# Meowuu7/equi-articulated-pose

Measured on AMD Instinct MI355X. Metric: point-clouds/sec (4096 pts, 60 anchors) fwd+bwd, higher is better.
Workload: dtype f32; 1 GPU; 8 x 4096-pt synthetic laptop clouds per GPU, 3-block inter backbone 1->64->128->512 (NN=64,K=24,A=60), forward+backward+Adam; clouds_per_gpu=8, points=4096, anchors=60

## Files before the change

equi-articulated-pose_amd/csrc/so3_dense.hip:

```cpp
#include <atomic>
#include "common.h"
#include "device_prims.h"
#include <type_traits>

namespace {

typedef unsigned long long u64;
typedef const __attribute__((address_space(4))) unsigned long long *cu64p;

constexpr int KC_BK = 32;
constexpr int KC_LIST_BYTES = 4096;

__host__ __device__ __forceinline__ void dense_kr(int d, int ks, int &k, int &r) {
    const int g = d / (16 * ks), rem = d - g * 16 * ks;
    k = rem >> 4;
    r = 16 * g + (rem & 15);
}


__device__ __forceinline__ void split2(float x0, float x1, unsigned &h, unsigned &l) {
    asm("v_cvt_pk_f16_f32 %0, %2, %3\n\t"
        "v_fma_mixlo_f16 %1, %0, -1.0, %2 op_sel:[0,0,0] op_sel_hi:[1,0,0]\n\t"
        "v_fma_mixhi_f16 %1, %0, -1.0, %3 op_sel:[1,0,0] op_sel_hi:[1,0,0]"
        : "=&v"(h), "=&v"(l) : "v"(x0), "v"(x1));
}

__global__ __launch_bounds__(256) void dense_slots_kernel(int n_sup, int rp, int rows_ld, const int32_t *__restrict__ rows,
                                                          const int32_t *__restrict__ n_rows, int32_t *__restrict__ slot_of) {
    const int b = blockIdx.y, j = blockIdx.x * 256 + threadIdx.x;
    if (j >= min(n_rows[b], rp)) return;
    const int r = rows[(size_t)b * rows_ld + j];
    if ((unsigned)r < (unsigned)n_sup) slot_of[(size_t)b * n_sup + r] = j;
}

constexpr int MEMB_WORDS = 16;
constexpr int MEMB_WORDS_WIDE = 32;
constexpr int DENSE_MAX_ROWS = 32 * MEMB_WORDS_WIDE;
template <int W>
__global__ __launch_bounds__(256) void dense_member_kernel(int p, int n_sup, int nn, int rp, const int32_t *__restrict__ idx,
                                                           const int32_t *__restrict__ slot_of, unsigned *__restrict__ memb,
                                                           int32_t *__restrict__ flags) {
    __shared__ unsigned sw[256][W + 1];
    const int b = blockIdx.y, pt = blockIdx.x * 256 + threadIdx.x;
    if (pt >= p) return;
    unsigned *w = sw[threadIdx.x];
    for (int k = 0; k < W; ++k) w[k] = 0u;
    const int32_t *list = idx + ((size_t)b * p + pt) * nn;
    int valid = 0, bad = 0;
    for (int n = 0; n < nn; ++n) {
        const int i = list[n];
        if ((unsigned)i >= (unsigned)n_sup) continue;
        const int s = slot_of[(size_t)b * n_sup + i];
        if (s < 0 || s >= rp) { bad |= 2; continue; }
        ++valid;
        w[s >> 5] |= 1u << (s & 31);
    }
    int bits = 0;
    for (int k = 0; k < W; ++k) { bits += __popc(w[k]); memb[((size_t)b * p + pt) * W + k] = w[k]; }
    if (bits != valid) bad |= 1;
    if (bad) atomicOr(&flags[b], bad);
}

template <int W>
__global__ __launch_bounds__(256) void dense_mask_kernel(int p, int ks, int rp, int dir, int wtiles, int steps,
                                                         const unsigned *__restrict__ memb, unsigned *__restrict__ bits) {
    const int b = blockIdx.y, lane = threadIdx.x & 63, li = lane & 31, kg = lane >> 5;
    const long long wv = (long long)blockIdx.x * 4 + (threadIdx.x >> 6);
    if (wv >= (long long)wtiles * steps) return;
    const int wt = (int)(wv / steps), step = (int)(wv - (long long)wt * steps);
    const int nkr = ks * rp;
    unsigned word = 0;
    if (dir == 0 && (ks & 3) == 0) {
        const int g = (64 * wt) / (16 * ks), pt_own = 32 * step + li;
        const unsigned own = (pt_own < p && 2 * (g >> 1) < 2 * W) ? memb[((size_t)b * p + pt_own) * W + (g >> 1)] : 0u;
        const int sh = 16 * (g & 1) + (li & 15);
        const bool col0 = 64 * wt + li < nkr, col1 = 64 * wt + 32 + li < nkr;
#pragma unroll
        for (int tt = 0; tt < 2; ++tt)
#pragma unroll
            for (int e = 0; e < 8; ++e) {
                const unsigned wd = (unsigned)__shfl((int)own, 16 * tt + 8 * kg + e);
                const unsigned bit = (wd >> sh) & 1u;
                word |= (col0 ? bit : 0u) << (16 * tt + e);
                word |= (col1 ? bit : 0u) << (16 * tt + 8 + e);
            }
    } else if (dir == 1) {
        const int d0 = 32 * step, g = d0 / (16 * ks);
#pragma unroll
        for (int j = 0; j < 2; ++j) {
            const int pt = 64 * wt + 32 * j + li;
            const unsigned wd = (pt < p && (g >> 1) < W) ? memb[((size_t)b * p + pt) * W + (g >> 1)] : 0u;
            const unsigned byte = (wd >> (16 * (g & 1) + 8 * kg)) & 0xffu;
#pragma unroll
            for (int tt = 0; tt < 2; ++tt)
                if (d0 + 16 * tt < nkr) word |= byte << (16 * tt + 8 * j);
        }
    } else {
#pragma unroll
        for (int i = 0; i < 32; ++i) {
            const int tt = i >> 4, j = (i >> 3) & 1, e = i & 7;
            const int n = 64 * wt + 32 * j + (lane & 31);
            const int kk = 32 * step + 16 * tt + 8 * (lane >> 5) + e;
            const int pt = dir ? n : kk, kr = dir ? kk : n;
            if (pt < p && kr < nkr) {
                int k_, r;
                dense_kr(kr, ks, k_, r);
                word |= ((memb[((size_t)b * p + pt) * W + (r >> 5)] >> (r & 31)) & 1u) << i;
            }
        }
    }
    bits[(((size_t)b * wtiles + wt) * steps + step) * 64 + lane] = word;
}

template <int W>
__global__ __launch_bounds__(256) void dense_keys_kernel(long long total, const unsigned *__restrict__ memb,
                                                         std::conditional_t<W == MEMB_WORDS, int32_t, int64_t> *__restrict__ keys) {
    using UK = std::conditional_t<W == MEMB_WORDS, unsigned, u64>;
    const long long i = (long long)blockIdx.x * 256 + threadIdx.x;
    if (i >= total) return;
    const u32x4 *w = reinterpret_cast<const u32x4 *>(memb + i * W);
    UK key = 0;
#pragma unroll
    for (int q = 0; q < W / 4; ++q) {
        const u32x4 v = w[q];
#pragma unroll
        for (int e = 0; e < 4; ++e) {
            const int g = 2 * (4 * q + e);
            key |= (UK)((v[e] & 0xffffu) ? 1u : 0u) << g;
            key |= (UK)((v[e] >> 16) ? 1u : 0u) << (g + 1);
        }
    }
    keys[i] = (std::conditional_t<W == MEMB_WORDS, int32_t, int64_t>)key;
}

__global__ __launch_bounds__(256) void dense_steps_kernel(int KS, int blocks_n, int wtiles, int dir, int ks, int row_slots, int skip,
                                                          const int32_t *__restrict__ n_rows, const unsigned *__restrict__ bits,
                                                          int32_t *__restrict__ steps) {
    extern __shared__ int nz[];
    const int b = blockIdx.y, bn = blockIdx.x, t = threadIdx.x, lane = t & 63, wave = t >> 6;
    for (int i = t; i < KS; i += 256) nz[i] = 0;
    __syncthreads();
    int limit = KS;
    if (dir == 1 && n_rows != nullptr) limit = max(min(KS, ((min(n_rows[b], row_slots) + 15) & ~15) * ks / KC_BK), 1);
    if (skip) {
        const int wt = min(4 * bn + wave, wtiles - 1);
        const unsigned *src = bits + ((size_t)b * wtiles + wt) * (size_t)KS * 64 + lane;
        for (int s = 0; s < limit; s += 4) {
            unsigned v[4];
#pragma unroll
            for (int u = 0; u < 4; ++u) v[u] = (s + u < limit) ? src[(size_t)(s + u) * 64] : 0u;
#pragma unroll
            for (int u = 0; u < 4; ++u)
                if (__builtin_amdgcn_ballot_w64(v[u] != 0u) != 0ull && lane == 0 && s + u < limit) nz[s + u] = 1;
        }
    } else {
        for (int i = t; i < limit; i += 256) nz[i] = 1;
    }
    __syncthreads();
    if (t == 0) {
        int32_t *dst = steps + ((size_t)b * blocks_n + bn) * (size_t)(KS + 1);
        int n = 0;
        for (int i = 0; i < KS; ++i)
            if (nz[i]) dst[1 + n++] = i;
        if (n == 0) dst[1 + n++] = 0;
        dst[0] = n;
    }
}

__global__ __launch_bounds__(256) void dense_centre_kernel(int n, const float *__restrict__ xyz, float *__restrict__ centre) {
    __shared__ double s[3][256];
    const int b = blockIdx.x;
// ... 318 lines not shown
                        v[4 + e] = hi ? own : got;
                    }
                    const int r0 = rc0 + 32 * rt + 16 * half + 8 * kg;
                    if (r0 < rc0 + nrows) {
                        unsigned h[4], l[4];
#pragma unroll
                        for (int e = 0; e < 4; ++e) split2(v[2 * e], v[2 * e + 1], h[e], l[e]);
                        const int kb = (r0 >> 4) * ks + k;
                        u32x4 *dst = planes + (((size_t)z * kb_total + kb) * MT + mt) * 128 + li + 32 * kg;
                        dst[0] = (u32x4){h[0], h[1], h[2], h[3]};
                        dst[64] = (u32x4){l[0], l[1], l[2], l[3]};
                    }
                }
            }
        }
    }
}

__global__ __launch_bounds__(256) void dense_untranspose_kernel(int nb, int o_total, int p, int na, int p_dst, const int32_t *__restrict__ map,
                                                                const int32_t *__restrict__ pivot_pos,
                                                                const float *__restrict__ yt, float *__restrict__ y,
                                                                float *__restrict__ psum, float *__restrict__ psq) {
    extern __shared__ float tile[];
    __shared__ float red[2][256];
    const int chunks = (p + 63) >> 6, t = threadIdx.x;
    const int p0 = (int)(blockIdx.x % (unsigned)chunks) * 64, grp_ = (int)(blockIdx.x / (unsigned)chunks), o = grp_ % o_total, b = grp_ / o_total;
    const int nchunk_x = chunks, nb_z = nb;
    const int np = min(64, p - p0);
    const float pivot = psum ? yt[(size_t)o * p + (pivot_pos ? *pivot_pos : 0)] : 0.f;
    float s = 0.f, q = 0.f;
    for (int i = t; i < na * 64; i += 256) {
        const int a = i >> 6, pp = i & 63;
        if (pp < np) {
            const float v = yt[(((size_t)b * na + a) * o_total + o) * p + p0 + pp];
            tile[a * 65 + pp] = v;
            if (psum != nullptr && (map == nullptr || map[(size_t)b * p + p0 + pp] >= 0)) {
                const float d = v - pivot;
                s += d; q = fmaf(d, d, q);
            }
        }
    }
    red[0][t] = s; red[1][t] = q;
    __syncthreads();
    const int nq = na >> 2;
    float *rows_y = y + ((size_t)b * o_total + o) * (size_t)(map ? p_dst : p) * na;
    for (int i = t; i < np * nq; i += 256) {
        const int pp = i / nq, a4 = i - pp * nq;
        const int q = map ? map[(size_t)b * p + p0 + pp] : p0 + pp;
        if (map != nullptr && (unsigned)q >= (unsigned)p_dst) continue;
        const float *src = tile + (4 * a4) * 65 + pp;
        const f32x4 v = {src[0], src[65], src[130], src[195]};
        *reinterpret_cast<f32x4 *>(rows_y + (size_t)q * na + 4 * a4) = v;
    }
    if (psum == nullptr) return;
    for (int h = 128; h > 0; h >>= 1) {
        if (t < h) { red[0][t] += red[0][t + h]; red[1][t] += red[1][t + h]; }
        __syncthreads();
    }
    if (t == 0) {
        const size_t at = ((size_t)o * nb_z + b) * nchunk_x + (p0 >> 6);
        psum[at] = red[0][0]; psq[at] = red[1][0];
    }
}

constexpr int UT_PTS = 128;
__global__ __launch_bounds__(256, 5) void dense_untranspose_tile_kernel(int o_total, int p, int na, int p_dst, const int32_t *__restrict__ map,
                                                                     const float *__restrict__ yt, float *__restrict__ y,
                                                                     const float *__restrict__ bn_scale, const float *__restrict__ bn_shift, float slope) {
    constexpr int UT_LD = UT_PTS / 16;
    extern __shared__ float tile[];
    __shared__ int dst_row[UT_PTS];
    const int chunks = (p + UT_PTS - 1) / UT_PTS, t = threadIdx.x;
    unsigned bid = blockIdx.x;
    if (const unsigned n8 = gridDim.x / 8u; bid < 8u * n8) bid = (bid % 8u) * n8 + bid / 8u;
    const int p0 = (int)(bid % (unsigned)chunks) * UT_PTS, grp_ = (int)(bid / (unsigned)chunks), o = grp_ % o_total, b = grp_ / o_total;
    const int np = min(UT_PTS, p - p0);
    if (t < UT_PTS) dst_row[t] = t >= np ? -1 : map ? map[(size_t)b * p + p0 + t] : p0 + t;
    const size_t a_pitch = (size_t)o_total * p;
    const float *src = yt + ((size_t)b * na * o_total + o) * p + p0;
    if ((p & 3) == 0) {
        f32x4 v[UT_LD];
#pragma unroll
        for (int k = 0; k < UT_LD; ++k) {
            const int i = t + 256 * k, a = i / (UT_PTS / 4), c = 4 * (i % (UT_PTS / 4));
            if (a < na && c < np) v[k] = *reinterpret_cast<const f32x4 *>(src + (size_t)a * a_pitch + c);
        }
#pragma unroll
        for (int k = 0; k < UT_LD; ++k) {
            const int i = t + 256 * k, a = i / (UT_PTS / 4), c = 4 * (i % (UT_PTS / 4));
            if (a < na && c < np) *reinterpret_cast<f32x4 *>(tile + a * UT_PTS + ((c + 4 * ((a >> 2) & 7)) & (UT_PTS - 1))) = v[k];
        }
    } else {
        for (int i = t; i < na * UT_PTS; i += 256) {
            const int a = i / UT_PTS, c = i % UT_PTS;
            if (c < np) tile[a * UT_PTS + ((c + 4 * ((a >> 2) & 7)) & (UT_PTS - 1))] = src[(size_t)a * a_pitch + c];
        }
    }
    __syncthreads();
    const int nq = na >> 2, RG = 256 / nq, a4 = t % nq, rr = t / nq;
    if (rr >= RG) return;
    const int rows_dst = map ? p_dst : p, rot = 4 * (a4 & 7);
    const float *quad = tile + (4 * a4) * UT_PTS;
    float *rows_y = y + ((size_t)b * o_total + o) * (size_t)rows_dst * na + 4 * a4;
    float sc = 1.f, sh = 0.f;
    if (bn_scale != nullptr) { sc = bn_scale[o]; sh = bn_shift[o]; }
    for (int pp0 = rr; pp0 < np; pp0 += 4 * RG) {
        f32x4 v[4];
        int q[4];
#pragma unroll
        for (int u = 0; u < 4; ++u) {
            const int pp = min(pp0 + u * RG, UT_PTS - 1), c = (pp + rot) & (UT_PTS - 1);
            q[u] = pp0 + u * RG < np ? dst_row[pp] : -1;
            v[u] = (f32x4){quad[c], quad[UT_PTS + c], quad[2 * UT_PTS + c], quad[3 * UT_PTS + c]};
        }
#pragma unroll
        for (int u = 0; u < 4; ++u) {
            if ((unsigned)q[u] >= (unsigned)rows_dst) continue;
            if (bn_scale != nullptr) {
#pragma unroll
                for (int e = 0; e < 4; ++e) { const float w = fmaf(v[u][e], sc, sh); v[u][e] = w > 0.f ? w : w * slope; }
            }
            *reinterpret_cast<f32x4 *>(rows_y + (size_t)q[u] * na) = v[u];
        }
    }
}

__global__ __launch_bounds__(256) void dense_zero_tail_kernel(int rows_ok, int na, int rp, long long ldz, const int32_t *__restrict__ n_rows,
                                                              float *__restrict__ z) {
    const int b = blockIdx.y, row = blockIdx.x;
    const int r0 = (min(n_rows[b], rp) + 15) & ~15, tail = rp - r0;
    if (tail <= 0) return;
    float *dst = z + ((long long)b * rows_ok + row) * ldz;
    for (int e = threadIdx.x; e < na * tail; e += 256) {
        const int a = e / tail;
        dst[(long long)a * rp + r0 + (e - a * tail)] = 0.f;
    }
}

struct KcArgs {
    int MT, N, KS, na, zcount;
    int tiles_m, blocks_n, mask_tiles;
    const u32x4 *A;
    const float *scale;
    const f32x4 *strT; long long strB, strA;
    const f32x4 *colT; long long colB, colA;
    const unsigned *mask;
    float neg_inv_sigma;
    const int32_t *n_rows; int ks, trim;
    float *C; long long cB, cA, ldm; int rp; long long kstride;
    int row_slots;
    const int32_t *steps;
};

template <int MI>
__global__ __launch_bounds__(256, MI == 4 ? 2 : 1) void kc_gemm_kernel(KcArgs g) {
    static_assert(MI == 8 || MI == 4, "the DMA piece schedule below: 8 or 4 KB of the stored operand per wave and k-step");
    constexpr unsigned WB = MI * 1024u;
    constexpr unsigned SUB_A = MI * 2048u;
    constexpr unsigned STR_OFF = 2 * SUB_A;
    constexpr unsigned BIT_OFF = STR_OFF + 1024u;
    constexpr unsigned STAGE = BIT_OFF + 1024u;
    extern __shared__ __attribute__((aligned(16))) unsigned char smem[];

    const int per_z = g.tiles_m * g.blocks_n;
    int id = blockIdx.x, z, local;
    {
        const int groups = g.zcount / 8 * 8;
        if (id < groups * per_z) {
            const int xcd = id & 7, slot = id >> 3;
            z = (slot / per_z) * 8 + xcd;
            local = slot % per_z;
        } else {
            const int r = id - groups * per_z;
            z = groups + r / per_z;
            local = r % per_z;
        }
    }
    const int bm = local % g.tiles_m, bn = local / g.tiles_m;
    const int b = z / g.na, a = z - b * g.na;
    const int used = (g.trim == 1 || g.trim == 2) ? ((min(g.n_rows[b], g.row_slots) + 15) & ~15) * g.ks : 0;
    const int N = g.trim == 1 ? min(g.N, used) : g.N;
    if (256 * bn >= N) return;
    const int32_t *lstG = g.steps ? g.steps + ((size_t)b * g.blocks_n + bn) * (size_t)(g.KS + 1) : nullptr;
    const int KS = lstG ? __builtin_amdgcn_readfirstlane(lstG[0]) : (g.trim == 2 ? max(min(g.KS, used / KC_BK), 1) : g.KS);
    int *lstL = reinterpret_cast<int *>(smem + 4 * STAGE);
    if (lstG != nullptr) {
        for (int i = threadIdx.x; i < KS; i += 256) lstL[i] = lstG[1 + i];
        __syncthreads();
    }
    auto step_at = [&](int i) __attribute__((always_inline)) { return lstG ? __builtin_amdgcn_readfirstlane(lstL[i]) : i; };

    const int t = threadIdx.x, lane = t & 63, li = lane & 31, kg = lane >> 5;
    const int wave = __builtin_amdgcn_readfirstlane(t >> 6);
    const int wt = bn * 4 + wave;
    const bool active = 64 * wt < N;

    const f32x4 *colz = g.colT + b * g.colB + a * g.colA;
    f32x4 cc[2];
#pragma unroll
    for (int j = 0; j < 2; ++j) cc[j] = colz[min(64 * wt + 32 * j + li, N - 1)];
    const float nis = g.neg_inv_sigma;

    const unsigned char *Aw = reinterpret_cast<const unsigned char *>(g.A) + ((size_t)z * 2 * g.KS * g.MT + (size_t)bm * MI) * 2048u
                              + (size_t)(wave >> 1) * ((size_t)g.MT * 2048u) + (size_t)(wave & 1) * WB;
    const size_t step_bytes = (size_t)g.MT * 4096u;
    const unsigned char *strw = reinterpret_cast<const unsigned char *>(g.strT + b * g.strB + a * g.strA) + (size_t)(wave & 1) * 256u;
    const unsigned char *bitw = reinterpret_cast<const unsigned char *>(g.mask) + ((size_t)b * g.mask_tiles + min(wt, g.mask_tiles - 1)) * (size_t)g.KS * 256u;
    const unsigned lds0 = lds_addr(smem);
    const unsigned ldsA = lds0 + (unsigned)(wave >> 1) * SUB_A + (unsigned)(wave & 1) * WB;
    const unsigned voff16 = (unsigned)lane * 16u, voff4 = (unsigned)lane * 4u;
#define DMA2(src, dst, o0, o1) asm volatile("s_mov_b32 m0, %2\n\ts_nop 0\n\tglobal_load_lds_dwordx4 %0, %1 offset:" #o0 "\n\tglobal_load_lds_dwordx4 %0, %1 offset:" #o1 \
                                            :: "v"(voff16), "s"(src), "s"(dst) : "memory")
#define DMA1(src, dst, o0) asm volatile("s_mov_b32 m0, %2\n\ts_nop 0\n\tglobal_load_lds_dwordx4 %0, %1 offset:" #o0 :: "v"(voff16), "s"(src), "s"(dst) : "memory")
#define DMA4B(src, dst) asm volatile("s_mov_b32 m0, %2\n\ts_nop 0\n\tglobal_load_lds_dword %0, %1" :: "v"(voff4), "s"(src), "s"(dst) : "memory")
    struct StepSrc { const unsigned char *a, *str, *bit; };
    auto src_of = [&](int step) __attribute__((always_inline)) {
        return StepSrc{Aw + (size_t)step * step_bytes, strw + (size_t)step * 512u, bitw + (size_t)step * 256u};
    };
    auto dma_slot = [&](const StepSrc &ss, unsigned stage_off, int slot) __attribute__((always_inline)) {
        const unsigned char *src = ss.a;
        const unsigned dst = ldsA + stage_off;
        if constexpr (MI == 8) {
            if (slot == 0) DMA2(src, dst, 0, 1024);
            if (slot == 1) DMA2(src, dst, 2048, 3072);
            if (slot == 2) DMA1(src + 4096, dst + 4096u, 0);
            if (slot == 3) DMA2(src + 4096, dst + 4096u, 1024, 2048);
            if (slot == 4) DMA1(src + 4096, dst + 4096u, 3072);
        } else {
            if (slot == 0) DMA2(src, dst, 0, 1024);
            if (slot == 2) DMA1(src, dst, 2048);
            if (slot == 3) DMA1(src, dst, 3072);
        }
        if (slot == 5) {
            DMA4B(ss.str, lds0 + stage_off + STR_OFF + (unsigned)wave * 256u);
            DMA4B(ss.bit, lds0 + stage_off + BIT_OFF + (unsigned)wave * 256u);
        }
    };
    auto issue = [&](int step, unsigned stage_off) __attribute__((always_inline)) {
        const StepSrc ss = src_of(step);
#pragma unroll
        for (int slot = 0; slot < 6; ++slot) dma_slot(ss, stage_off, slot);
    };

    f32x16 acc[MI][2];
#pragma unroll
    for (int i = 0; i < MI; ++i)
#pragma unroll
        for (int j = 0; j < 2; ++j)
#pragma unroll
            for (int r = 0; r < 16; ++r) acc[i][j][r] = 0.f;

    constexpr bool LEAN = MI == 4;
    typedef float f32x3 __attribute__((ext_vector_type(3)));
    using SV = std::conditional_t<LEAN, f32x3, f32x4>;
    struct BFrag { u32x4 h[2], l[2]; };
    auto frag_a = [&](const unsigned char *st, int sub, int plane, u32x4 (&f)[MI]) __attribute__((always_inline)) {
#pragma unroll
        for (int i = 0; i < MI; ++i) f[i] = *reinterpret_cast<const u32x4 *>(st + (unsigned)sub * SUB_A + (unsigned)(2 * i + plane) * 1024u + (unsigned)lane * 16u);
    };
    auto gen2 = [&](const SV (&sv)[8], unsigned mb, int tb, int j, int e0, BFrag &f) __attribute__((always_inline)) {
        float v[2];
#pragma unroll
        for (int e = 0; e < 2; ++e) {
            const SV s = sv[e0 + e];
            const int keep = (int)(mb << (31 - (16 * tb + 8 * j + e0 + e))) >> 31;
            const float one = __int_as_float(keep & 0x3f800000);
            const float tx = cc[j].x - s.x, ty = cc[j].y - s.y, tz = cc[j].z - s.z;
            const float d2 = fmaf(tz, tz, fmaf(ty, ty, tx * tx));
            v[e] = __builtin_amdgcn_fmed3f(fmaf(d2, nis, one), 0.f, 1.f);
        }
        unsigned h, l;
        split2(v[0], v[1], h, l);
        f.h[j][e0 / 2] = h;
        f.l[j][e0 / 2] = l;
    };
    auto load_sv = [&](const f32x4 *str, SV (&sv)[8]) __attribute__((always_inline)) {
#pragma unroll
        for (int e = 0; e < 8; ++e) sv[e] = *reinterpret_cast<const SV *>(str + 8 * kg + e);
    };
    auto mm = [&](const u32x4 &fa, const u32x4 &fb, f32x16 &c) __attribute__((always_inline)) {
        c = __builtin_amdgcn_mfma_f32_32x32x16_f16(__builtin_bit_cast(f16x8, fa), __builtin_bit_cast(f16x8, fb), c, 0, 0, 0);
    };
#define SB() __builtin_amdgcn_sched_barrier(0)
#define PIPE_HALF(NV, ND)                                                         \
    _Pragma("unroll") for (int i_ = 0; i_ < MI; ++i_) {                           \
        __builtin_amdgcn_sched_group_barrier(0x008, 1, 0);                        \
        if constexpr ((ND) > 0) __builtin_amdgcn_sched_group_barrier(0x100, (ND) > 0 ? (ND) : 1, 0);  \
        __builtin_amdgcn_sched_group_barrier(0x002, NV, 0);                       \
    }
#define PIPE(NV, ND0, ND1) PIPE_HALF(NV, ND0) PIPE_HALF(NV, ND1)
    auto kblock = [&](const unsigned char *st, int sub, const unsigned char *nst, int nsub, const f32x4 *nnstr, unsigned mb, int tb,
                      const BFrag &Bc, BFrag &Bn, u32x4 (&ah)[MI], const SV (&sv)[8], SV (&nsv)[8], auto dma) __attribute__((always_inline)) {
        u32x4 al[MI];
        constexpr int NV1 = MI == 8 ? 4 : 7, NV3 = MI == 8 ? 3 : 5;
        SB();
        frag_a(st, sub, 1, al);
        if constexpr (!LEAN) load_sv(nnstr, nsv);
        dma(0);
#pragma unroll
        for (int i = 0; i < MI; ++i) { mm(ah[i], Bc.h[0], acc[i][0]); mm(ah[i], Bc.h[1], acc[i][1]); }
        gen2(sv, mb, tb, 0, 0, Bn); gen2(sv, mb, tb, 0, 2, Bn); gen2(sv, mb, tb, 0, 4, Bn);
        if constexpr (LEAN) { PIPE(NV1, 1, 0) } else { PIPE(NV1, (MI == 8 ? 1 : 2), 1) }
        SB();
        dma(1);
#pragma unroll
        for (int i = 0; i < MI; ++i) { mm(ah[i], Bc.l[0], acc[i][0]); mm(ah[i], Bc.l[1], acc[i][1]); }
        gen2(sv, mb, tb, 0, 6, Bn); gen2(sv, mb, tb, 1, 0, Bn); gen2(sv, mb, tb, 1, 2, Bn);
        PIPE(NV1, 0, 0)
        SB();
        frag_a(nst, nsub, 0, ah);
        dma(2);
#pragma unroll
        for (int i = 0; i < MI; ++i) { mm(al[i], Bc.h[0], acc[i][0]); mm(al[i], Bc.h[1], acc[i][1]); }
        gen2(sv, mb, tb, 1, 4, Bn); gen2(sv, mb, tb, 1, 6, Bn);
        PIPE(NV3, 1, 0)
        SB();
        if constexpr (LEAN) { load_sv(nnstr, nsv); SB(); }
    };

    const int last = KS - 1;
    issue(step_at(0), 0);
    issue(step_at(min(1, last)), STAGE);
    issue(step_at(min(2, last)), 2 * STAGE);
    int ahead = lstG ? lstL[min(3, last)] : 0;
    asm volatile("s_waitcnt vmcnt(0)" ::: "memory");
    __builtin_amdgcn_s_barrier();
    BFrag B0, B1;
    u32x4 ah[MI];
    SV sv[8], sw[8];
    unsigned mbc = *reinterpret_cast<const unsigned *>(smem + BIT_OFF + (unsigned)t * 4u);
    {
        load_sv(reinterpret_cast<const f32x4 *>(smem + STR_OFF), sv);
#pragma unroll
        for (int e = 0; e < 8; e += 2) { gen2(sv, mbc, 0, 0, e, B0); gen2(sv, mbc, 0, 1, e, B0); }
        frag_a(smem, 0, 0, ah);
        load_sv(reinterpret_cast<const f32x4 *>(smem + STR_OFF) + 16, sv);
    }

    unsigned s0 = 0, s1 = STAGE, s2 = 2 * STAGE, s3 = 3 * STAGE;
    for (int s = 0; s < KS; ++s) {
        if (s > 0) {
            if constexpr (MI == 8) asm volatile("s_waitcnt vmcnt(10)" ::: "memory");
            else asm volatile("s_waitcnt vmcnt(6)" ::: "memory");
            __builtin_amdgcn_s_barrier();
        }
        const int nxt = lstG ? __builtin_amdgcn_readfirstlane(ahead) : min(s + 3, last);
        const StepSrc ssn = src_of(nxt);
        if (lstG != nullptr) ahead = lstL[min(s + 4, last)];
        const unsigned dst = s3;
        const unsigned mbn = *reinterpret_cast<const unsigned *>(smem + s1 + BIT_OFF + (unsigned)t * 4u);
        const f32x4 *str1 = reinterpret_cast<const f32x4 *>(smem + s1 + STR_OFF);
        kblock(smem + s0, 0, smem + s0, 1, str1, mbc, 1, B0, B1, ah, sv, LEAN ? sv : sw, [&](int slot) __attribute__((always_inline)) {
            dma_slot(ssn, dst, slot);
        });
        kblock(smem + s0, 1, smem + s1, 0, str1 + 16, mbn, 0, B1, B0, ah, LEAN ? sv : sw, sv, [&](int slot) __attribute__((always_inline)) {
            dma_slot(ssn, dst, 3 + slot);
        });
        mbc = mbn;
        { const unsigned r = s0; s0 = s1; s1 = s2; s2 = s3; s3 = r; }
    }
#undef SB
#undef PIPE
#undef PIPE_HALF
#undef DMA1
#undef DMA2
#undef DMA4B

    asm volatile("s_waitcnt vmcnt(0)" ::: "memory");
    __syncthreads();
    float *isc = reinterpret_cast<float *>(smem);
    if (t < 32 * MI) isc[t] = 1.0f / g.scale[(size_t)z * (32 * g.MT) + 32 * MI * bm + t];
    __syncthreads();
    if (!active) return;
    float *Cz = g.C + b * g.cB + a * g.cA + (long long)(32 * MI * bm) * g.ldm;
#pragma unroll
    for (int j = 0; j < 2; ++j) {
        const int n = 64 * wt + 32 * j + li;
        if (n >= N) continue;
        int k = n / g.rp, r = n - k * g.rp;
        if (g.trim & 1) dense_kr(n, g.ks, k, r);
        const long long coff = (long long)k * g.kstride + r;
#pragma unroll
        for (int i = 0; i < MI; ++i)
#pragma unroll
            for (int r = 0; r < 16; ++r) {
                const int row = 32 * i + (r & 3) + 8 * (r >> 2) + 4 * kg;
                Cz[(long long)row * g.ldm + coff] = acc[i][j][r] * isc[row];
            }
    }
}

template <int MI>
int kc_launch(const KcArgs &g, hipStream_t s) {
    constexpr size_t shmem = 4 * (2 * (size_t)MI * 2048u + 2048u) + KC_LIST_BYTES;
    eap::set_kernel(MI == 8 ? "kc_gemm_kernel<8, 1>" : "kc_gemm_kernel<4, 1>");
    return eap::run_kernel("so3_dense product", kc_gemm_kernel<MI>, (long long)g.zcount * g.tiles_m * g.blocks_n, 1, 1, dim3(256), shmem, s, g);
}

inline int ceil_to(int v, int q) { return (v + q - 1) / q * q; }

}

namespace {
inline bool dense_shape_ok(int p, int na, int ks, int rp, int o, int words) {
    return p > 0 && (p % 32) == 0 && na > 0 && (na % 4) == 0 && na <= 64 && ks > 0 && (ks % 2) == 0 && rp > 0 && (rp % 16) == 0 && rp <= 32 * words &&
           (o % 128) == 0;
}
}

extern "C" int eap_so3_dense_supported(int p, int na, int ks, int rp, int o) { return dense_shape_ok(p, na, ks, rp, o, MEMB_WORDS_WIDE); }

extern "C" int eap_so3_dense_max_rows(void) { return DENSE_MAX_ROWS; }

extern "C" int64_t eap_so3_dense_mask_words(int b, int p, int ks, int rp, int dir) {
    const int n = dir ? p : ks * rp, kd = dir ? ceil_to(ks * rp, KC_BK) : p;
    const int wtiles = 4 * ((n + 255) / 256), steps = kd / KC_BK;
    return ((int64_t)b * wtiles * steps * 64 + 1) / 2;
}

namespace {
template <int W>
int dense_member(int b, int p, int n_sup, int nn, int rp, int rows_ld, const int32_t *idx, const int32_t *rows, const int32_t *n_rows, int32_t *slot_of,
                 uint32_t *memb, int32_t *flags, eap_stream_t stream) {
    if (b <= 0 || p <= 0) return 0;
    if (rp <= 0 || rp > 32 * W) return eap::bad_arg(W == MEMB_WORDS ? "so3_dense_member: 0 < rp <= 512" : "so3_dense_member_wide: 0 < rp <= 1024");
    hipStream_t s = eap::S(stream);
    if (int e = eap::hip_fail(hipMemsetAsync(slot_of, 0xff, sizeof(int32_t) * (size_t)b * n_sup, s), "so3_dense_member memset")) return e;
    if (int e = eap::hip_fail(hipMemsetAsync(flags, 0, sizeof(int32_t) * (size_t)b, s), "so3_dense_member memset")) return e;
    if (int e = eap::run_kernel("so3_dense_member", dense_slots_kernel, eap::cdiv(rp, 256), b, 1, dim3(256), 0, s, n_sup, rp, rows_ld, rows, n_rows, slot_of)) return e;
    return eap::run_kernel("so3_dense_member", dense_member_kernel<W>, eap::cdiv(p, 256), b, 1, dim3(256), 0, s, p, n_sup, nn, rp, idx, slot_of, memb, flags);
}

template <int W>
int dense_masks(int b, int p, int ks, int rp, int dir, const uint32_t *memb, uint64_t *mask, eap_stream_t stream) {
    if (b <= 0) return 0;
    if (!dense_shape_ok(p, 4, ks, rp, 256, W)) return eap::bad_arg("so3_dense_masks: shape not taken");
    const int n = dir ? p : ks * rp, kd = dir ? ceil_to(ks * rp, KC_BK) : p;
    const int wtiles = 4 * ((n + 255) / 256), steps = kd / KC_BK;
    return eap::run_kernel("so3_dense_masks", dense_mask_kernel<W>, eap::cdiv((long long)wtiles * steps, 4), b, 1, dim3(256), 0, eap::S(stream), p, ks, rp, dir, wtiles, steps,
                           memb, reinterpret_cast<unsigned *>(mask));
}
}

extern "C" int eap_so3_dense_member(int b, int p, int n_sup, int nn, int rp, int rows_ld, const int32_t *idx, const int32_t *rows,
                                    const int32_t *n_rows, int32_t *slot_of, uint32_t *memb, int32_t *flags, eap_stream_t stream) {
    return dense_member<MEMB_WORDS>(b, p, n_sup, nn, rp, rows_ld, idx, rows, n_rows, slot_of, memb, flags, stream);
}

extern "C" int eap_so3_dense_member_wide(int b, int p, int n_sup, int nn, int rp, int rows_ld, const int32_t *idx, const int32_t *rows,
                                         const int32_t *n_rows, int32_t *slot_of, uint32_t *memb, int32_t *flags, eap_stream_t stream) {
    return dense_member<MEMB_WORDS_WIDE>(b, p, n_sup, nn, rp, rows_ld, idx, rows, n_rows, slot_of, memb, flags, stream);
}

extern "C" int eap_so3_dense_masks(int b, int p, int ks, int rp, int dir, const uint32_t *memb, uint64_t *mask, eap_stream_t stream) {
    return dense_masks<MEMB_WORDS>(b, p, ks, rp, dir, memb, mask, stream);
}

extern "C" int eap_so3_dense_masks_wide(int b, int p, int ks, int rp, int dir, const uint32_t *memb, uint64_t *mask, eap_stream_t stream) {
    return dense_masks<MEMB_WORDS_WIDE>(b, p, ks, rp, dir, memb, mask, stream);
}

extern "C" int eap_so3_dense_tables_f32(int b, int p, int n_sup, int na, int ks, int rp, int rows_ld, float sigma, const float *q_xyz,
                                        const float *s_xyz, const int32_t *rows, const float *rk, const float *row_rot, float *centre, float *pt,
                                        float *kr, eap_stream_t stream) {
    if (b <= 0) return 0;
    if (!(sigma > 0.f)) return eap::bad_arg("so3_dense_tables: sigma > 0");
    hipStream_t s = eap::S(stream);
    const int p_pad = ceil_to(p, KC_BK), kd_pad = ceil_to(ks * rp, KC_BK);
    if (int e = eap::run_kernel("so3_dense_tables", dense_centre_kernel, b, 1, 1, dim3(256), 0, s, n_sup, s_xyz, centre)) return e;
    if (int e = eap::run_kernel("so3_dense_tables", dense_points_kernel, eap::cdiv(p_pad, 256), b, 1, dim3(256), 0, s, p, p_pad, q_xyz, centre,
                                reinterpret_cast<f32x4 *>(pt)))
        return e;
    return eap::run_kernel("so3_dense_tables", dense_rows_kernel, eap::cdiv(kd_pad, 256), na, b, dim3(256), 0, s, n_sup, na, ks, rp, kd_pad, rows_ld,
                           s_xyz, centre, rows, rk, row_rot, reinterpret_cast<f32x4 *>(kr));
}

extern "C" int eap_so3_dense_split_f32(int b, int m, int l, int na, int seg, int64_t seg_pitch, int mapped, const int32_t *n_rows, const uint32_t *rowmax,
                                       const int32_t *colmap, const float *src, float *scale, void *planes, eap_stream_t stream) {
    if (b <= 0) return 0;
    if (colmap != nullptr) {
        if (mapped || seg_pitch <= 0 || (l & 7) != 0 || (reinterpret_cast<uintptr_t>(colmap) & 15) != 0)
            return eap::bad_arg("so3_dense_split: a column map (16-byte aligned, a multiple of 8 columns) comes with the source row pitch and without the dense-index mapping");
        seg = l;
    }
    if (seg <= 0) { seg = l; seg_pitch = (int64_t)l * na; }
    if ((m % 32) != 0 || (na % 4) != 0 || na > 64 || (reinterpret_cast<uintptr_t>(src) & 15) || l % seg != 0 ||
        (seg_pitch & 3) != 0 || (colmap == nullptr && seg_pitch < (int64_t)seg * na) || (mapped && ((seg % 16) != 0 || ((l / seg) % 2) != 0)))
        return eap::bad_arg("so3_dense_split: m % 32, na % 4, na <= 64, 16-byte aligned source, whole segments of a 16-byte aligned pitch (mapped: seg % 16, an even number of segments)");
    if ((colmap ? (int64_t)1 : (int64_t)(l / seg)) * (seg_pitch / 4) > 0x7fffffffLL) return eap::bad_arg("so3_dense_split: a source row of at most 2^31 16-byte pieces");
    hipStream_t s = eap::S(stream);
    const int kb_total = ceil_to(l, KC_BK) / 16;
    float *scale2 = scale + (size_t)b * na * m;
    const int e = rowmax != nullptr
                      ? eap::run_kernel("so3_dense_split", dense_scale_kernel, eap::cdiv((long long)b * m * na, 256), 1, 1, dim3(256), 0, s, (long long)b * m * na, m, na, rowmax, scale, scale2)
                      : eap::run_kernel("so3_dense_split", dense_rowmax_kernel, m, b, 1, dim3(256), 0, s, m, l, na, seg, (long long)(seg_pitch / 4), colmap,
                                        reinterpret_cast<const f32x4 *>(src), scale, scale2);
    if (e) return e;
    return eap::run_kernel("so3_dense_split", dense_split_kernel<false>, (long long)kb_total * (m / 32) * b * 2, 1, 1, dim3(256), (size_t)na * 1024, s, m, l, na, kb_total, seg, (long long)(seg_pitch / 4),
                           mapped ? 1 : 0, n_rows, colmap, reinterpret_cast<const f32x4 *>(src), scale2, reinterpret_cast<u32x4 *>(planes), SplitBn{nullptr, nullptr, 1.f, 1.f});
}

extern "C" int eap_so3_dense_split_bn_f32(int b, int m, int l, int l_src, int na, const uint32_t *rowbound, const int32_t *colmap, const float *grad,
                                          const float *act, const float *coef, float slope, float *scale, void *planes, eap_stream_t stream) {
    if (b <= 0) return 0;
    if (colmap == nullptr && l != l_src) return eap::bad_arg("so3_dense_split_bn: without a column map l = l_src");
    if ((m % 32) != 0 || (na % 4) != 0 || na > 64 || ((reinterpret_cast<uintptr_t>(grad) | reinterpret_cast<uintptr_t>(act)) & 15) ||
        (colmap != nullptr && ((l & 7) != 0 || (reinterpret_cast<uintptr_t>(colmap) & 15) != 0)) || rowbound == nullptr || coef == nullptr || !(slope > 0.f))
        return eap::bad_arg("so3_dense_split_bn: m % 32, na % 4, na <= 64, 16-byte aligned sources, a bound per row, a positive slope (column map: 16-byte aligned, l % 8)");
    if ((int64_t)l_src * na / 4 > 0x7fffffffLL) return eap::bad_arg("so3_dense_split_bn: a source row of at most 2^31 16-byte pieces");
    hipStream_t s = eap::S(stream);
    const int kb_total = ceil_to(l, KC_BK) / 16;
    float *scale2 = scale + (size_t)b * na * m;
    if (int e = eap::run_kernel("so3_dense_split_bn", dense_scale_kernel, eap::cdiv((long long)b * m * na, 256), 1, 1, dim3(256), 0, s, (long long)b * m * na, m, na, rowbound, scale,
                                scale2))
        return e;
    const int seg = colmap ? l : l_src;
    return eap::run_kernel("so3_dense_split_bn", dense_split_kernel<true>, (long long)kb_total * (m / 32) * b * 2, 1, 1, dim3(256), (size_t)na * 1024, s, m, l, na, kb_total, seg,
                           (long long)l_src * na / 4, 0, nullptr, colmap, reinterpret_cast<const f32x4 *>(grad), scale2, reinterpret_cast<u32x4 *>(planes),
                           SplitBn{reinterpret_cast<const f32x4 *>(act), coef, slope, 1.0f / slope});
}

namespace {
int untranspose_args(const char *what, int o, int p, int na, const float *yt, const float *y) {
    char buf[256];
    const char *why = nullptr;
    if (o <= 0 || p <= 0) why = "o > 0 and p > 0";
    else if (na <= 0 || (na % 4) != 0) why = "na % 4 == 0 (rows of Y are stored as 16-byte pieces)";
    else if (na > 64) why = "na <= 64 (the tile of a block)";
    else if (yt == nullptr || (reinterpret_cast<uintptr_t>(yt) & 15) != 0) why = "yt 16-byte aligned";
    else if (y == nullptr || (reinterpret_cast<uintptr_t>(y) & 15) != 0) why = "y 16-byte aligned";
    if (why == nullptr) return 0;
    snprintf(buf, sizeof(buf), "%s: %s", what, why);
    return eap::bad_arg(buf);
}

int untranspose_tile(const char *what, int b, int o, int p, int na, int p_dst, const int32_t *map, const float *yt, float *y, const float *bn_scale,
                     const float *bn_shift, float slope, eap_stream_t stream) {
    return eap::run_kernel(what, dense_untranspose_tile_kernel, (long long)eap::cdiv(p, UT_PTS) * o * b, 1, 1, dim3(256), sizeof(float) * (size_t)na * UT_PTS,
                           eap::S(stream), o, p, na, p_dst, map, yt, y, bn_scale, bn_shift, slope);
}
}

extern "C" int eap_so3_dense_untranspose_bnact_f32(int b, int o, int p, int na, int p_dst, const int32_t *map, const float *yt, const float *bn_scale,
                                                   const float *bn_shift, float slope, float *y, eap_stream_t stream) {
    if (b <= 0) return 0;
    if (bn_scale == nullptr || bn_shift == nullptr || (map != nullptr && p_dst <= 0) || (map == nullptr && p_dst != p))
        return eap::bad_arg("so3_dense_untranspose_bnact: scale and shift per channel; p_dst = p without a map");
    if (int e = untranspose_args("so3_dense_untranspose_bnact", o, p, na, yt, y)) return e;
    return untranspose_tile("so3_dense_untranspose_bnact", b, o, p, na, p_dst, map, yt, y, bn_scale, bn_shift, slope, stream);
}

extern "C" int eap_so3_dense_gplanes_supported(int o, int c, int na, int ks, int rp) {
    return (o % 32) == 0 && (c == 64 || c == 128) && na > 0 && ks > 0 && (ks % 2) == 0 && rp > 0 && (rp % 16) == 0;
}

extern "C" int eap_so3_dense_gplanes_f32(int b, int o, int c, int na, int ks, int rp, const float *W3, const float *Ft, const int32_t *n_rows,
                                         const float *bound, float *scale, void *planes, eap_stream_t stream) {
    if (b <= 0) return 0;
    if (!eap_so3_dense_gplanes_supported(o, c, na, ks, rp) ||
        ((reinterpret_cast<uintptr_t>(W3) | reinterpret_cast<uintptr_t>(Ft) | reinterpret_cast<uintptr_t>(planes)) & 15) != 0)
        return eap::bad_arg("so3_dense_gplanes: shape not taken (eap_so3_dense_gplanes_supported), 16-byte aligned operands");
    const int kb_total = ceil_to(ks * rp, KC_BK) / 16;
    const int fit = (int)((84u * 1024u) / ((size_t)(2 * c + 16) * 2)) / 16 * 16;
    const int rch = min(rp, max(fit, 32));
    const size_t shmem = (size_t)rch * (2 * c + 16) * 2;
    return eap::run_kernel("so3_dense_gplanes", c == 128 ? dense_gplanes_kernel<8> : dense_gplanes_kernel<4>, eap::cdiv(o / 32, 4), (long long)b * na, 1, dim3(256), shmem,
                           eap::S(stream), o, na, ks, rp, rch, kb_total, W3, Ft, n_rows, bound, scale, reinterpret_cast<u32x4 *>(planes));
}

extern "C" int eap_so3_dense_product_steps_f32(int dir, int b, int o, int p, int na, int ks, int rp, int64_t ldz, float sigma, const int32_t *n_rows,
                                               const void *planes, const float *scale, const float *pt, const float *kr, const uint64_t *mask,
                                               const int32_t *steps, float *out, eap_stream_t stream) {
    if (b <= 0) return 0;
    if (!eap_so3_dense_supported(p, na, ks, rp, o)) return eap::bad_arg("so3_dense_product: shape not taken (eap_so3_dense_supported)");
    const int p_pad = ceil_to(p, KC_BK), kd_pad = ceil_to(ks * rp, KC_BK);
    KcArgs g;
    g.MT = o / 32; g.na = na; g.zcount = b * na; g.row_slots = rp;
    g.N = dir ? p : ks * rp;
    g.KS = (dir ? kd_pad : p) / KC_BK;
    const bool wide = (o % 256) == 0;
    g.tiles_m = wide ? o / 256 : o / 128;
    g.blocks_n = (g.N + 255) / 256;
    g.mask_tiles = 4 * g.blocks_n;
    g.A = reinterpret_cast<const u32x4 *>(planes);
    g.scale = scale;
    const f32x4 *ptT = reinterpret_cast<const f32x4 *>(pt), *krT = reinterpret_cast<const f32x4 *>(kr);
    if (dir == 0) {
        g.strT = ptT; g.strB = p_pad; g.strA = 0;
        g.colT = krT; g.colB = (long long)na * kd_pad; g.colA = kd_pad;
        if (ldz < (int64_t)na * rp) return eap::bad_arg("so3_dense_product: ldz < na rp");
        g.cB = (long long)o * ks * ldz; g.cA = rp; g.ldm = (long long)ks * ldz; g.rp = rp; g.kstride = ldz;
    } else {
        g.strT = krT; g.strB = (long long)na * kd_pad; g.strA = kd_pad;
        g.colT = ptT; g.colB = p_pad; g.colA = 0;
        g.cB = (long long)na * o * p; g.cA = (long long)o * p; g.ldm = p; g.rp = p; g.kstride = 0;
    }
    g.mask = reinterpret_cast<const unsigned *>(mask);
    g.steps = (steps != nullptr && g.KS <= KC_LIST_BYTES / 4) ? steps : nullptr;
    g.C = out;
    g.neg_inv_sigma = -1.0f / sigma;
    g.n_rows = n_rows; g.ks = ks; g.trim = dir ? 2 : 1;
    if (n_rows == nullptr) g.trim = dir ? 0 : 3;
    if (dir == 0 && n_rows != nullptr) {
        if (int e = eap::run_kernel("so3_dense zero tail", dense_zero_tail_kernel, (long long)o * ks, b, 1, dim3(256), 0, eap::S(stream), o * ks, na, rp, (long long)ldz, n_rows, out))
            return e;
    }
    return wide ? kc_launch<8>(g, eap::S(stream)) : kc_launch<4>(g, eap::S(stream));
}

extern "C" int eap_so3_dense_product_f32(int dir, int b, int o, int p, int na, int ks, int rp, int64_t ldz, float sigma, const int32_t *n_rows,
                                         const void *planes, const float *scale, const float *pt, const float *kr, const uint64_t *mask, float *out, eap_stream_t stream) {
    return eap_so3_dense_product_steps_f32(dir, b, o, p, na, ks, rp, ldz, sigma, n_rows, planes, scale, pt, kr, mask, nullptr, out, stream);
}

extern "C" int eap_so3_dense_point_keys(int b, int p, const uint32_t *memb, int32_t *keys, eap_stream_t stream) {
    if (b <= 0 || p <= 0) return 0;
    const long long total = (long long)b * p;
    return eap::run_kernel("so3_dense_point_keys", dense_keys_kernel<MEMB_WORDS>, eap::cdiv(total, 256), 1, 1, dim3(256), 0, eap::S(stream), total, memb, keys);
}

extern "C" int eap_so3_dense_point_keys_wide(int b, int p, const uint32_t *memb, int64_t *keys, eap_stream_t stream) {
    if (b <= 0 || p <= 0) return 0;
    const long long total = (long long)b * p;
    return eap::run_kernel("so3_dense_point_keys_wide", dense_keys_kernel<MEMB_WORDS_WIDE>, eap::cdiv(total, 256), 1, 1, dim3(256), 0, eap::S(stream), total, memb, keys);
}

extern "C" int64_t eap_so3_dense_steps_words(int b, int p, int ks, int rp, int dir) {
    const int n = dir ? p : ks * rp, kd = dir ? ceil_to(ks * rp, KC_BK) : p;
    return (int64_t)b * ((n + 255) / 256) * (kd / KC_BK + 1);
}

namespace {
int dense_steps(int words, int b, int p, int ks, int rp, int dir, int skip, const int32_t *n_rows, const uint64_t *mask, int32_t *steps, eap_stream_t stream) {
    if (b <= 0) return 0;
    if (!dense_shape_ok(p, 4, ks, rp, 256, words)) return eap::bad_arg("so3_dense_steps: shape not taken");
    const int n = dir ? p : ks * rp, kd = dir ? ceil_to(ks * rp, KC_BK) : p;
    const int blocks_n = (n + 255) / 256, KS = kd / KC_BK;
    if ((size_t)KS * sizeof(int) > 48 * 1024) return eap::bad_arg("so3_dense_steps: more than 12288 k-steps");
    return eap::run_kernel("so3_dense_steps", dense_steps_kernel, blocks_n, b, 1, dim3(256), sizeof(int) * (size_t)KS, eap::S(stream), KS, blocks_n, 4 * blocks_n, dir, ks, rp, skip,
                           n_rows, reinterpret_cast<const unsigned *>(mask), steps);
}
}

extern "C" int eap_so3_dense_steps(int b, int p, int ks, int rp, int dir, int skip, const int32_t *n_rows, const uint64_t *mask, int32_t *steps,
                                   eap_stream_t stream) {
    return dense_steps(MEMB_WORDS, b, p, ks, rp, dir, skip, n_rows, mask, steps, stream);
}

extern "C" int eap_so3_dense_steps_wide(int b, int p, int ks, int rp, int dir, int skip, const int32_t *n_rows, const uint64_t *mask, int32_t *steps,
                                        eap_stream_t stream) {
    return dense_steps(MEMB_WORDS_WIDE, b, p, ks, rp, dir, skip, n_rows, mask, steps, stream);
}

extern "C" int eap_so3_dense_untranspose_f32(int b, int o, int p, int na, const float *yt, float *y, float *psum, float *psq, eap_stream_t stream) {
    if (b <= 0) return 0;
    if (int e = untranspose_args("so3_dense_untranspose", o, p, na, yt, y)) return e;
    if (psum == nullptr) return untranspose_tile("so3_dense_untranspose", b, o, p, na, p, nullptr, yt, y, nullptr, nullptr, 1.f, stream);
    if (psq == nullptr) return eap::bad_arg("so3_dense_untranspose: both partial arrays or neither");
    return eap::run_kernel("so3_dense_untranspose", dense_untranspose_kernel, (long long)eap::cdiv(p, 64) * o * b, 1, 1, dim3(256), sizeof(float) * (size_t)na * 65, eap::S(stream), b, o, p, na,
                           p, nullptr, nullptr, yt, y, psum, psq);
}

extern "C" int eap_so3_dense_untranspose_map_f32(int b, int o, int p, int na, int p_dst, const int32_t *map, const float *yt, float *y,
                                                 eap_stream_t stream) {
    if (b <= 0) return 0;
    if (map == nullptr || p_dst <= 0) return eap::bad_arg("so3_dense_untranspose_map: a map, p_dst > 0");
    if (int e = untranspose_args("so3_dense_untranspose_map", o, p, na, yt, y)) return e;
    return untranspose_tile("so3_dense_untranspose_map", b, o, p, na, p_dst, map, yt, y, nullptr, nullptr, 1.f, stream);
}

extern "C" int eap_so3_dense_untranspose_map_stats_f32(int b, int o, int p, int na, int p_dst, const int32_t *map, const int32_t *pivot_pos, const float *yt,
                                                       float *y, float *psum, float *psq, eap_stream_t stream) {
    if (b <= 0) return 0;
    if (map == nullptr || pivot_pos == nullptr || p_dst <= 0 || psum == nullptr || psq == nullptr)
        return eap::bad_arg("so3_dense_untranspose_map_stats: a map, the pivot column, both partial arrays");
    if (int e = untranspose_args("so3_dense_untranspose_map_stats", o, p, na, yt, y)) return e;
    return eap::run_kernel("so3_dense_untranspose_map_stats", dense_untranspose_kernel, (long long)eap::cdiv(p, 64) * o * b, 1, 1, dim3(256), sizeof(float) * (size_t)na * 65, eap::S(stream), b, o, p, na,
                           p_dst, map, pivot_pos, yt, y, psum, psq);
}
```

Baseline: 168.4 point-clouds/sec.

## Add 16x16x32 MFMA body with hand-scheduled interleaved kernel-weight generation

Adds a specialised path of the dense SO(3) kernel-correlation GEMM for the 256-row block. It uses v_mfma_f32_16x16x32_f16 in place of the 32x32 MFMA and fully unrolls each k-step into compile-time slots. Each slot interleaves one MFMA with DMA issue, LDS fragment reads and the split-f16 Gaussian weight computation for the next step, separated by scheduling barriers. The aim is to hide the VALU weight generation and LDS traffic behind matrix instructions. In exchange it adds heavy code growth and register pressure, plus a permlane16 swap in the epilogue to restore the output layout.

```diff
diff --git a/equi-articulated-pose_amd/csrc/so3_dense.hip b/equi-articulated-pose_amd/csrc/so3_dense.hip
--- a/equi-articulated-pose_amd/csrc/so3_dense.hip
+++ b/equi-articulated-pose_amd/csrc/so3_dense.hip
@@ -2,6 +2,7 @@
 #include "common.h"
 #include "device_prims.h"
 #include <type_traits>
+#include <utility>
 
 namespace {
 
@@ -17,6 +18,11 @@
     r = 16 * g + (rem & 15);
 }
 
+
+template <int... Is, class F>
+__device__ __forceinline__ void static_for(std::integer_sequence<int, Is...>, F &&f) {
+    (f(std::integral_constant<int, Is>{}), ...);
+}
 
 __device__ __forceinline__ void split2(float x0, float x1, unsigned &h, unsigned &l) {
     asm("v_cvt_pk_f16_f32 %0, %2, %3\n\t"
@@ -641,9 +647,10 @@
     const int32_t *steps;
 };
 
-template <int MI>
+template <int MI, bool M16>
 __global__ __launch_bounds__(256, MI == 4 ? 2 : 1) void kc_gemm_kernel(KcArgs g) {
     static_assert(MI == 8 || MI == 4, "the DMA piece schedule below: 8 or 4 KB of the stored operand per wave and k-step");
+    static_assert(!M16 || MI == 8, "the 16x16x32 body is cut for the 256-row block: eight regions of two row tiles per k-step");
     constexpr unsigned WB = MI * 1024u;
     constexpr unsigned SUB_A = MI * 2048u;
     constexpr unsigned STR_OFF = 2 * SUB_A;
@@ -731,6 +738,165 @@
         for (int slot = 0; slot < 6; ++slot) dma_slot(ss, stage_off, slot);
     };
 
+    if constexpr (M16) {
+        constexpr int RT = 2 * MI;
+        const int c16 = lane & 15, q = lane >> 4;
+        f32x4 cq[4];
+#pragma unroll
+        for (int jt = 0; jt < 4; ++jt) cq[jt] = colz[min(64 * wt + 16 * jt + c16, N - 1)];
+        const unsigned aoff = (unsigned)(q >> 1) * SUB_A + (unsigned)((q & 1) * 32 + c16) * 16u;
+        const unsigned soff = STR_OFF + (unsigned)q * 128u;
+        const unsigned boff = BIT_OFF + (unsigned)wave * 256u + (unsigned)((q & 1) * 32 + c16) * 4u;
+        const unsigned msh = 16u * (unsigned)(q >> 1);
+
+        f32x4 acc[RT][4];
+#pragma unroll
+        for (int i = 0; i < RT; ++i)
+#pragma unroll
+            for (int j = 0; j < 4; ++j)
+#pragma unroll
+                for (int r = 0; r < 4; ++r) acc[i][j][r] = 0.f;
+        struct BFrag { u32x4 h[4], l[4]; };
+        struct AFrag { u32x4 h, l; };
+        struct Side { f32x4 sv[8]; unsigned mbe, mbo; };
+        auto side_read = [&](const unsigned char *st, int i, Side &sd) __attribute__((always_inline)) {
+            if (i == 0) sd.mbe = *reinterpret_cast<const unsigned *>(st + boff);
+            else if (i == 9) sd.mbo = *reinterpret_cast<const unsigned *>(st + boff + 64u);
+            else sd.sv[i - 1] = *reinterpret_cast<const f32x4 *>(st + soff + 16u * (unsigned)(i - 1));
+        };
+        auto side_bits = [&](unsigned &mb, unsigned keep) __attribute__((always_inline)) { mb = (mb >> msh) & keep; };
+        auto frag_read = [&](const unsigned char *st, int rt, int i, AFrag (&f)[2]) __attribute__((always_inline)) {
+            const int r = rt + (i >> 1);
+            const u32x4 x = *reinterpret_cast<const u32x4 *>(st + aoff + (unsigned)(r >> 1) * 2048u + (unsigned)(r & 1) * 256u + (unsigned)(i & 1) * 1024u);
+            if (i & 1) f[i >> 1].l = x; else f[i >> 1].h = x;
+        };
+        struct WTmp { float tx, ty, tz, d2, one; int kb; };
+        WTmp wt4[4] = {};
+        float val[2][4] = {{0.f, 0.f, 0.f, 0.f}, {0.f, 0.f, 0.f, 0.f}};
+        unsigned hh[2] = {0, 0}, ll[2] = {0, 0};
+        auto vop = [&](auto oc, const Side &sd, BFrag &f) __attribute__((always_inline)) {
+            constexpr int O = decltype(oc)::value;
+            const float nv = nis;
+            if constexpr (O >= 0 && O < 342) {
+                constexpr int t = O < 336 ? O / 42 : 8, at = O < 336 ? O % 42 : (O - 336 < 2 ? 4 : O - 336 < 4 ? 14 : 24) + (O & 1);
+                if constexpr (at == 4 || at == 5 || at == 14 || at == 15 || at == 24 || at == 25) {
+                    if constexpr (t > 0) {
+                        constexpr int j = at & 1, pp = 2 * (t - 1) + j, jt = pp >> 2, wd = pp & 3;
+                        const float x0 = val[(t - 1) & 1][2 * j], x1 = val[(t - 1) & 1][2 * j + 1];
+                        if constexpr (at < 6) asm volatile("v_cvt_pk_f16_f32 %0, %1, %2" : "=v"(hh[j]) : "v"(x0), "v"(x1));
+                        else if constexpr (at < 16) asm volatile("v_fma_mixlo_f16 %0, %1, -1.0, %2 op_sel:[0,0,0] op_sel_hi:[1,0,0]" : "=v"(ll[j]) : "v"(hh[j]), "v"(x0));
+                        else {
+                            asm volatile("v_fma_mixhi_f16 %0, %1, -1.0, %2 op_sel:[1,0,0] op_sel_hi:[1,0,0]" : "+v"(ll[j]) : "v"(hh[j]), "v"(x1));
+                            f.h[jt][wd] = hh[j];
+                            f.l[jt][wd] = ll[j];
+                        }
+                    }
+                } else if constexpr (t < 8) {
+                    constexpr int idx = at - (at > 24 ? 6 : at > 14 ? 4 : at > 4 ? 2 : 0);
+                    constexpr int i = idx & 3, k = idx >> 2, pr = 2 * t + (i >> 1), jt = pr >> 2, e = 2 * (pr & 3) + (i & 1), bit = 8 * (jt >> 1) + e;
+                    WTmp &w = wt4[i];
+                    const f32x4 sk = sd.sv[e];
+                    const unsigned mb = (jt & 1) ? sd.mbo : sd.mbe;
+                    if constexpr (k == 0) asm volatile("v_sub_f32 %0, %1, %2" : "=v"(w.tx) : "v"(cq[jt].x), "v"(sk.x));
+                    if constexpr (k == 1) asm volatile("v_sub_f32 %0, %1, %2" : "=v"(w.ty) : "v"(cq[jt].y), "v"(sk.y));
+                    if constexpr (k == 2) asm volatile("v_sub_f32 %0, %1, %2" : "=v"(w.tz) : "v"(cq[jt].z), "v"(sk.z));
+                    if constexpr (k == 3) asm volatile("v_mul_f32 %0, %1, %1" : "=v"(w.d2) : "v"(w.tx));
+                    if constexpr (k == 4) asm volatile("v_fmac_f32 %0, %1, %1" : "+v"(w.d2) : "v"(w.ty));
+                    if constexpr (k == 5) asm volatile("v_fmac_f32 %0, %1, %1" : "+v"(w.d2) : "v"(w.tz));
+                    if constexpr (k == 6) asm volatile("v_bfe_i32 %0, %1, %2, 1" : "=v"(w.kb) : "v"(mb), "n"(bit));
+                    if constexpr (k == 7) asm volatile("v_and_b32 %0, 1.0, %1" : "=v"(w.one) : "v"(w.kb));
+                    if constexpr (k == 8) asm volatile("v_fma_f32 %0, %1, %2, %3 clamp" : "=v"(val[t & 1][i]) : "v"(w.d2), "s"(nv), "v"(w.one));
+                }
+            }
+        };
+        auto slot = [&](auto mc, const unsigned char *st, const unsigned char *nst, unsigned keep, AFrag (&Ae)[2], AFrag (&Ao)[2], const BFrag &Bc,
+                        BFrag &Bn, Side &sd, auto dma) __attribute__((always_inline)) {
+            constexpr int M = decltype(mc)::value, G = M / 24, w = M % 24, h = w / 12, prod = (w % 12) / 4, jt = w % 4;
+            __builtin_amdgcn_sched_barrier(0);
+            AFrag (&Ac)[2] = (G & 1) ? Ao : Ae;
+            AFrag (&An)[2] = (G & 1) ? Ae : Ao;
+            const u32x4 &fa = prod < 2 ? Ac[h].h : Ac[h].l, &fb = prod == 1 ? Bc.l[jt] : Bc.h[jt];
+            asm volatile("v_mfma_f32_16x16x32_f16 %0, %1, %2, %0" : "+a"(acc[2 * G + h][jt]) : "v"(fa), "v"(fb));
+            if constexpr (w == 0 && G < 6) dma(G);
+            if constexpr (G == 0 && w < 10) side_read(nst, w, sd);
+            constexpr int ar = G == 0 ? w - 10 : w;
+            if constexpr (ar >= 0 && ar < 4) frag_read(G == MI - 1 ? nst : st, (2 * G + 2) % RT, ar, An);
+            if constexpr (M == 18) side_bits(sd.mbe, keep);
+            if constexpr (M == 19) side_bits(sd.mbo, keep);
+            vop(std::integral_constant<int, 2 * (M - 20)>{}, sd, Bn);
+            vop(std::integral_constant<int, 2 * (M - 20) + 1>{}, sd, Bn);
+            __builtin_amdgcn_sched_barrier(0);
+        };
+
+        const int last = KS - 1;
+        issue(step_at(0), 0);
+        issue(step_at(min(1, last)), STAGE);
+        issue(step_at(min(2, last)), 2 * STAGE);
+        int ahead = lstG ? lstL[min(3, last)] : 0;
+        asm volatile("s_waitcnt vmcnt(0)" ::: "memory");
+        __builtin_amdgcn_s_barrier();
+        BFrag B0, B1;
+        AFrag A0[2], A1[2];
+        Side sd;
+#pragma unroll
+        for (int i = 0; i < 10; ++i) side_read(smem, i, sd);
+        side_bits(sd.mbe, ~0u);
+        side_bits(sd.mbo, ~0u);
+#pragma unroll
+        for (int i = 0; i < 4; ++i) frag_read(smem, 0, i, A0);
+
+        unsigned s0 = 0, s1 = STAGE, s2 = 2 * STAGE, s3 = 3 * STAGE;
+        auto kstep = [&](int s, const BFrag &Bc, BFrag &Bn) __attribute__((always_inline)) {
+            if (s > 0) {
+                asm volatile("s_waitcnt vmcnt(10)" ::: "memory");
+                __builtin_amdgcn_s_barrier();
+            }
+            const int nxt = lstG ? __builtin_amdgcn_readfirstlane(ahead) : min(s + 3, last);
+            const StepSrc ssn = src_of(nxt);
+            if (lstG != nullptr) ahead = lstL[min(s + 4, last)];
+            const unsigned dst = s3;
+            const unsigned char *st = smem + s0, *nst = smem + s1;
+            const unsigned keep = s + 1 < KS ? ~0u : 0u;
+            auto dma = [&](int slot) __attribute__((always_inline)) { dma_slot(ssn, dst, slot); };
+            static_for(std::make_integer_sequence<int, 24 * MI>{}, [&](auto mc) __attribute__((always_inline)) { slot(mc, st, nst, keep, A0, A1, Bc, Bn, sd, dma); });
+            { const unsigned r = s0; s0 = s1; s1 = s2; s2 = s3; s3 = r; }
+        };
+        static_for(std::make_integer_sequence<int, 342>{}, [&](auto oc) __attribute__((always_inline)) { vop(oc, sd, B0); });
+        for (int s = 0; s < KS; s += 2) {
+            kstep(s, B0, B1);
+            kstep(s + 1, B1, B0);
+        }
+
+        asm volatile("s_nop 15\n\ts_waitcnt vmcnt(0)" ::: "memory");
+        __syncthreads();
+        float *isc = reinterpret_cast<float *>(smem);
+        if (t < 32 * MI) isc[t] = 1.0f / g.scale[(size_t)z * (32 * g.MT) + 32 * MI * bm + t];
+        __syncthreads();
+        if (!active) return;
+        float *Cz = g.C + b * g.cB + a * g.cA + (long long)(32 * MI * bm) * g.ldm;
+#pragma unroll
+        for (int jp = 0; jp < 2; ++jp) {
+            const int n = 64 * wt + 32 * jp + 16 * (q & 1) + c16;
+            const bool ok = n < N;
+            int k = n / g.rp, r = n - k * g.rp;
+            if (g.trim & 1) dense_kr(n, g.ks, k, r);
+            const long long coff = (long long)k * g.kstride + r;
+#pragma unroll
+            for (int i = 0; i < RT; ++i)
+#pragma unroll
+                for (int e = 0; e < 4; ++e) {
+                    const float sc = isc[16 * i + 4 * q + e];
+                    const auto sw = __builtin_amdgcn_permlane16_swap(__float_as_uint(acc[i][2 * jp][e] * sc), __float_as_uint(acc[i][2 * jp + 1][e] * sc), false, false);
+                    const int row = 16 * i + 4 * (q & ~1) + e;
+                    if (ok) {
+                        Cz[(long long)row * g.ldm + coff] = __uint_as_float(sw[0]);
+                        Cz[(long long)(row + 4) * g.ldm + coff] = __uint_as_float(sw[1]);
+                    }
+                }
+        }
+        return;
+    }
+
     f32x16 acc[MI][2];
 #pragma unroll
     for (int i = 0; i < MI; ++i)
@@ -879,11 +1045,13 @@
     }
 }
 
-template <int MI>
+constexpr bool kc_body16(int mi, int dir) { return mi == 8 && (dir == 0 || dir == 1); }
+
+template <int MI, int DIR>
 int kc_launch(const KcArgs &g, hipStream_t s) {
     constexpr size_t shmem = 4 * (2 * (size_t)MI * 2048u + 2048u) + KC_LIST_BYTES;
     eap::set_kernel(MI == 8 ? "kc_gemm_kernel<8, 1>" : "kc_gemm_kernel<4, 1>");
-    return eap::run_kernel("so3_dense product", kc_gemm_kernel<MI>, (long long)g.zcount * g.tiles_m * g.blocks_n, 1, 1, dim3(256), shmem, s, g);
+    return eap::run_kernel("so3_dense product", kc_gemm_kernel<MI, kc_body16(MI, DIR)>, (long long)g.zcount * g.tiles_m * g.blocks_n, 1, 1, dim3(256), shmem, s, g);
 }
 
 inline int ceil_to(int v, int q) { return (v + q - 1) / q * q; }
@@ -1094,7 +1262,8 @@
         if (int e = eap::run_kernel("so3_dense zero tail", dense_zero_tail_kernel, (long long)o * ks, b, 1, dim3(256), 0, eap::S(stream), o * ks, na, rp, (long long)ldz, n_rows, out))
             return e;
     }
-    return wide ? kc_launch<8>(g, eap::S(stream)) : kc_launch<4>(g, eap::S(stream));
+    if (wide) return dir ? kc_launch<8, 1>(g, eap::S(stream)) : kc_launch<8, 0>(g, eap::S(stream));
+    return dir ? kc_launch<4, 1>(g, eap::S(stream)) : kc_launch<4, 0>(g, eap::S(stream));
 }
 
 extern "C" int eap_so3_dense_product_f32(int dir, int b, int o, int p, int na, int ks, int rp, int64_t ldz, float sigma, const int32_t *n_rows,
```

Result: no change. 169.7 point-clouds/sec (median of 6 runs) (+0.8%).
